# MCG-NKU/E2FGVI

Measured on AMD Instinct MI355X. Metric: inpainted frames/sec at 432x240 T=10, higher is better.
Workload: dtype f32; 1 GPU; BASELINE.json configs[1]: e2fgvi 432x240 T=10 l_t=10, 1 clip(s) per GPU per forward (1 in the job), random-init weights, torch.rand frames + box mask (SURVEY.md 8d); clips_per_gpu=1, precision=fp32, kernel_selection=e2fgvi_amd/tile_table.py (checked in, deterministic: ops.py), hip_graph=True, forwards_in_flight=2

## Files before the change

### e2fgvi_amd/build.py

```python
import os
import subprocess
import sys
from concurrent.futures import ThreadPoolExecutor

HERE = os.path.dirname(os.path.abspath(__file__))
CSRC = os.path.join(HERE, "csrc")
LIB = os.path.join(CSRC, "libe2fgvi_hip.so")
FLAGS = ["--offload-arch=gfx950", "-O3", "-std=c++17", "-fPIC", "-ffp-contract=fast"]
NOPK = ["-Xclang", "-target-feature", "-Xclang", "-packed-fp32-ops"]
UNITS = [("error.hip", "error.o", []), ("conv.hip", "conv.o", []), ("conv.hip", "conv_nopk.o", NOPK + ["-DE2_NOPK_VARIANT"]),
         ("conv_bf16x.hip", "conv_bf16x.o", NOPK), ("conv_wino.hip", "conv_wino.o", NOPK), ("conv_wino.hip", "conv_wino_x3.o", NOPK + ["-DE2_WINO_X3=1"]), ("conv_wino4.hip", "conv_wino4.o", NOPK), ("conv_tail.hip", "conv_tail.o", NOPK),
         ("mdcn.hip", "mdcn.o", NOPK), ("attention.hip", "attention.o", []),
         ("attention_bf16.hip", "attention_bf16.o", NOPK), ("attention_x3.hip", "attention_x3.o", NOPK), ("misc.hip", "misc.o", NOPK),
         ("video.hip", "video.o", NOPK), ("metrics.hip", "metrics.o", NOPK)]
NOPK_OBJECTS = ("conv_nopk.o", "conv_bf16x.o", "conv_wino.o", "conv_wino4.o", "conv_wino_x3.o", "conv_tail.o", "mdcn.o", "attention_bf16.o", "attention_x3.o", "misc.o", "video.o", "metrics.o")
OBJDUMP = "/opt/rocm/lib/llvm/bin/llvm-objdump"


def _hipcc():
    for c in (os.environ.get("HIPCC"), "/opt/rocm/bin/hipcc"):
        if c and os.path.exists(c):
            return c
    return "hipcc"


def _stale(out, deps):
    return (not os.path.exists(out)) or any(os.path.getmtime(d) > os.path.getmtime(out) for d in deps)


def build(force=False, verbose=False, nopk_all=False, lib=None, tag=None, defines=()):
    hipcc = _hipcc()
    if tag:
        nopk_all = False
    objdir = os.path.join(CSRC, ("build_" + tag) if tag else ("build_nopk" if nopk_all else "build"))
    os.makedirs(objdir, exist_ok=True)
    out = lib or (os.path.join(CSRC, "libe2fgvi_hip_%s.so" % tag) if tag else
                  os.path.join(CSRC, "libe2fgvi_hip_nopk.so") if nopk_all else LIB)
    headers = [os.path.join(CSRC, "common.h"), os.path.join(HERE, "..", "include", "e2fgvi_hip.h"), os.path.abspath(__file__)]
    jobs = []
    for src, obj, extra in UNITS:
        sp, op = os.path.join(CSRC, src), os.path.join(objdir, obj)
        if nopk_all and not any(f == "-packed-fp32-ops" for f in extra):
            extra = extra + NOPK
        if force or _stale(op, [sp] + headers):
            jobs.append([hipcc] + FLAGS + extra + list(defines) + ["-c", sp, "-o", op])

    def run(cmd):
        if verbose:
            print(" ".join(cmd), flush=True)
        subprocess.check_call(cmd)

    with ThreadPoolExecutor(max_workers=min(4, max(1, len(jobs)))) as ex:
        list(ex.map(run, jobs))
    objs = [os.path.join(objdir, obj) for _, obj, _ in UNITS]
    if force or jobs or _stale(out, objs):
        run([hipcc, "--offload-arch=gfx950", "-shared", "-fPIC", "-o", out] + objs)
    if jobs:
        verify_isa(objdir)
        if not nopk_all:
            verify_wino_waits(objdir)
            verify_exit_reuse(objdir)
            verify_no_scratch(objdir)
    return out


def build_variant(tag, *defines):
    return build(tag=tag, defines=defines)


def device_isa(obj):
    import shutil
    import tempfile
    d = tempfile.mkdtemp(prefix="e2isa")
    try:
        local = os.path.join(d, os.path.basename(obj))
        shutil.copy(obj, local)
        subprocess.run([OBJDUMP, "--offloading", os.path.basename(obj)], cwd=d, check=True, stdout=subprocess.DEVNULL,
                       stderr=subprocess.DEVNULL)
        dev = [f for f in os.listdir(d) if "gfx950" in f]
        if not dev:
            return ""
        return subprocess.run([OBJDUMP, "-d", os.path.join(d, dev[0])], check=True, capture_output=True, text=True).stdout
    finally:
        shutil.rmtree(d, ignore_errors=True)


def verify_isa(objdir=None):
    import re
    objdir = objdir or os.path.join(CSRC, "build")
    if not os.path.exists(OBJDUMP):
        return
    for obj in NOPK_OBJECTS:
        isa = device_isa(os.path.join(objdir, obj))
        bad = re.findall(r"v_pk_(?:mul|add|fma)_f32", isa)
        if bad or not isa:
# ... 273 lines not shown
```

### e2fgvi_amd/csrc/common.h

```cpp
#pragma once
#include <hip/hip_runtime.h>
#include <stdint.h>
#include <stdio.h>
#include <stdarg.h>

#include "../../include/e2fgvi_hip.h"

typedef float f32x4 __attribute__((ext_vector_type(4)));
typedef float f32x16 __attribute__((ext_vector_type(16)));

void e2fgvi_set_error(const char* fmt, ...);

#define E2_REQUIRE(cond, code, ...)            \
    do {                                       \
        if (!(cond)) {                         \
            e2fgvi_set_error(__VA_ARGS__);     \
            return (code);                     \
        }                                      \
    } while (0)

#define E2_LAUNCH_CHECK(name)                                                        \
    do {                                                                             \
        hipError_t e__ = hipGetLastError();                                          \
        if (e__ != hipSuccess) {                                                     \
// ... 54 lines not shown
typedef __bf16 e2_bf16x8 __attribute__((ext_vector_type(8)));
typedef unsigned int e2_u32x4 __attribute__((ext_vector_type(4)));
__device__ __forceinline__ void e2_split8(const f32x4& v0, const f32x4& v1, e2_bf16x8& hi, e2_bf16x8& mid, e2_bf16x8& lo) {
    float x[8];
#pragma unroll
    for (int j = 0; j < 4; ++j) { x[j] = v0[j]; x[4 + j] = v1[j]; }
    e2_u32x4 H, M, L;
#pragma unroll
    for (int j = 0; j < 4; ++j) {
        unsigned h, m, l;
        e2_split2(x[2 * j], x[2 * j + 1], h, m, l);
        H[j] = h; M[j] = m; L[j] = l;
    }
    hi = __builtin_bit_cast(e2_bf16x8, H);
    mid = __builtin_bit_cast(e2_bf16x8, M);
    lo = __builtin_bit_cast(e2_bf16x8, L);
}

typedef _Float16 e2_f16x8 __attribute__((ext_vector_type(8)));
template <bool F16> struct e2_h16;
template <> struct e2_h16<false> { typedef __bf16 T; typedef e2_bf16x8 V8; };
template <> struct e2_h16<true> { typedef _Float16 T; typedef e2_f16x8 V8; };
__device__ __forceinline__ f32x16 e2_mfma16(e2_bf16x8 a, e2_bf16x8 b, f32x16 c) {
    return __builtin_amdgcn_mfma_f32_32x32x16_bf16(a, b, c, 0, 0, 0);
}
__device__ __forceinline__ f32x16 e2_mfma16(e2_f16x8 a, e2_f16x8 b, f32x16 c) {
    return __builtin_amdgcn_mfma_f32_32x32x16_f16(a, b, c, 0, 0, 0);
}
template <bool F16> __device__ __forceinline__ float e2_h16_to_f32(unsigned short b) {
    if constexpr (F16) return (float)__builtin_bit_cast(_Float16, b);
    else return __builtin_bit_cast(float, (unsigned)b << 16);
}

__device__ __forceinline__ float apply_act(float v, int act, float slope) {
    if (act == E2FGVI_ACT_RELU) return fmaxf(v, 0.f);
    if (act == E2FGVI_ACT_LRELU) return v > 0.f ? v : v * slope;
    if (act == E2FGVI_ACT_TANH) return tanhf(v);
    return v;
}
```

### e2fgvi_amd/csrc/conv_bf16x.hip

```cpp
#include "common.h"

namespace {

typedef __bf16 bf16x8 __attribute__((ext_vector_type(8)));
typedef unsigned int u32x4 __attribute__((ext_vector_type(4)));
typedef __attribute__((address_space(3))) void lds_void;

struct ConvXParams {
    const void* src[E2FGVI_MAX_SRC];
    int ld[E2FGVI_MAX_SRC];
    int coff[E2FGVI_MAX_SRC];
    int cpg[E2FGVI_MAX_SRC];
    unsigned src_bytes[E2FGVI_MAX_SRC];
    int nsrc;
    int N, H, W, Ho, Wo, KH, KW, stride, pad;
    int padx;
    int osy, osx, opy, opx, oH, oW;
    int res_bcast;
    int Cout, Cout_g, Npad;
    int M;
    int tilesM, tilesN;
    int nsteps;
    unsigned wgroup_bytes;
    long long wgroup_elems;
    const void* w;
    const float* bias;
    const void* res;
    int res_ld, res_coff, res_bf16;
    void* dst;
    int dst_ld, dst_coff, dst_bf16, dst_nchw;
    __bf16* dst2;
    int dst2_ld, dst2_coff;
    int split_from;
    long long split_plane;
    int act;
    float slope;
    int tp_cq;
    unsigned tp_magic;
    unsigned tp_magic_cq;
    int dbg_noload;
};

__device__ __forceinline__ __amdgpu_buffer_rsrc_t make_rsrc(const void* base, unsigned bytes) {
    return __builtin_amdgcn_make_buffer_rsrc(const_cast<void*>(base), 0, (int)bytes, 0x00020000);
}

__device__ __forceinline__ float dcn_post(float v, int co, int C, const f32x4& fl, float max_residue) {
    const int noff = (C / 3) * 2;
    if (co >= noff) return e2_fast_sigmoid(v);
    const int which = (co * 2 >= noff) ? 2 : 0;
    return max_residue * e2_fast_tanh(v) + fl[which + ((co & 1) ? 0 : 1)];
}


__device__ __forceinline__ void split8(const f32x4& v0, const f32x4& v1, bf16x8& hi, bf16x8& mid, bf16x8& lo) {
    e2_split8(v0, v1, hi, mid, lo);
}

typedef int pp_i32x4 __attribute__((ext_vector_type(4)));
__device__ __forceinline__ pp_i32x4 pp_rsrc_words(const void* base, unsigned bytes) {
    const unsigned long long b = (unsigned long long)base;
    pp_i32x4 r;
    r[0] = __builtin_amdgcn_readfirstlane((int)(unsigned)b);
    r[1] = __builtin_amdgcn_readfirstlane((int)((unsigned)(b >> 32) & 0xFFFFu));
    r[2] = __builtin_amdgcn_readfirstlane((int)bytes);
    r[3] = 0x00020000;
    return r;
}
__device__ __forceinline__ void pp_dma16(pp_i32x4 rsrc, unsigned lds_dst, unsigned voff, unsigned soff) {
    unsigned keep;
    asm volatile("s_nop 4\n\ts_mov_b32 %0, m0\n\ts_mov_b32 m0, %3\n\ts_nop 0\n\tbuffer_load_dwordx4 %1, %2, %4 offen lds\n\ts_mov_b32 m0, %0"
                 : "=&s"(keep) : "v"(voff), "s"(rsrc), "s"(lds_dst), "s"(soff) : "memory");
}

template <int BM, int BN, int WGM, int WGN, bool S3, int MODE, bool PP = false>
__global__ __launch_bounds__(64 * WGM * WGN) void conv_bf16x_kernel(const ConvXParams p) {
#if defined(__HIP_DEVICE_COMPILE__)
    constexpr bool F32 = MODE == 1, X3 = MODE == 2, F16 = MODE == 3;
    typedef typename e2_h16<F16>::T E16;
    typedef typename e2_h16<F16>::V8 e16x8;
    static_assert(!PP || (X3 && !S3 && WGM * WGN == 8), "ping-pong halves: split-operand mode, 8 waves, no row-shift stages");
    constexpr int NT = 64 * WGM * WGN;
    constexpr int ESZ = (F32 || X3) ? 4 : 2;
    constexpr int CH = 16 / ESZ;
    constexpr int KC = 8 * CH;
    constexpr int TM = BM / (32 * WGM), TN = BN / (32 * WGN);
    constexpr int AR = S3 ? BM + 2 : BM;
    constexpr int B_CH = X3 ? 12 : 8;
    constexpr int A_BYTES = AR * 128, B_BYTES = BN * B_CH * 16;
    constexpr int A_IT = (AR * 8 + NT - 1) / NT, B_IT = (BN * B_CH + NT - 1) / NT;
    constexpr bool A_PART = (AR * 8) % NT != 0;
    constexpr bool B_PART = (BN * B_CH) % NT != 0;
    constexpr int R = TM * 32, CN = TN * 32;
    constexpr int ES = (WGM * WGN * R * (CN + 4) * 4 <= 150 * 1024) ? 1 : (TN % 2 == 0 ? 2 : TN);
    constexpr int TNH = TN / ES, CNH = CN / ES, LDE = CNH + 4;
    constexpr int EPI = WGM * WGN * R * LDE * 4;
    static_assert(TN % ES == 0 && EPI <= 160 * 1024, "epilogue region");
    constexpr int SMEM = 2 * (A_BYTES + B_BYTES) > EPI ? 2 * (A_BYTES + B_BYTES) : EPI;
    constexpr unsigned OOB = 0xFFFFFFFFu;
    static_assert(TM >= 1 && TN >= 1 && (BM * 8) % NT == 0 && (BN * B_CH) % 64 == 0 && SMEM <= 160 * 1024, "tile");

    __shared__ __attribute__((aligned(1024))) unsigned char smem[SMEM];

    const int tid = threadIdx.x;
    const int lane = tid & 63, wave = __builtin_amdgcn_readfirstlane(tid >> 6);
// ... 886 lines not shown
    p.wgroup_elems = q.wgroup_elems; p.wgroup_bytes = (unsigned)(q.wgroup_elems * wbytes_num);
    p.w = d->wpacked; p.bias = d->bias;
    p.res = d->residual; p.res_ld = d->res_ld; p.res_coff = d->res_coff; p.res_bf16 = d->res_dtype == dt16;
    p.dst = d->dst; p.dst_ld = d->dst_ld; p.dst_coff = d->dst_coff; p.dst_bf16 = d->dst_dtype == dt16;
    p.dst_nchw = d->dst_nchw;
    p.dst2 = (__bf16*)d->dst2; p.dst2_ld = d->dst2_ld; p.dst2_coff = d->dst2_coff;
    p.split_from = d->dst2_split_from; p.split_plane = d->dst2_plane_stride;
    p.act = d->act; p.slope = d->slope;
    hipStream_t st = (hipStream_t)stream;
    int tile = d->tile;
    p.dbg_noload = 0;
    if (tile == 21 || tile == 24 || tile == 26 || tile == 27) { p.dbg_noload = 1; tile -= 20; }
    if (tile == 31 || tile == 34 || tile == 36) { p.dbg_noload = 2; tile -= 30; }
    if (tile == 41 || tile == 44 || tile == 46) { p.dbg_noload = 3; tile -= 40; }
    if (tile == 61 || tile == 66) { p.dbg_noload = 8; tile -= 60; }
    if (tile == 71 || tile == 74 || tile == 76 || tile == 77) { p.dbg_noload = 16; tile -= 70; }
    if (tile == 81 || tile == 84 || tile == 86 || tile == 87) { p.dbg_noload = 32; tile -= 80; }
    if (!tile) {
        if (p.Cout_g <= 32) tile = 3;
        else if (p.Cout_g <= 64) tile = 2;
        else tile = ((long long)cdiv(p.M, 128) * cdiv(p.Cout_g, 128) * d->groups >= 384) ? 1 : 4;
    }
    switch (tile) {
        case 1: return launch_x<128, 128, 2, 2, false>(p, d->groups, st, mode);
        case 2: return launch_x<128, 64, 2, 2, false>(p, d->groups, st, mode);
        case 3: return launch_x<128, 32, 4, 1, false>(p, d->groups, st, mode);
        case 4: return launch_x<64, 128, 2, 2, false>(p, d->groups, st, mode);
        case 5: return launch_x<64, 64, 2, 2, false>(p, d->groups, st, mode);
        case 6: return launch_x<256, 128, 4, 2, false>(p, d->groups, st, mode);
        case 7: return launch_x<256, 256, 4, 2, false>(p, d->groups, st, mode);
        case 8: return launch_x<256, 192, 4, 2, false>(p, d->groups, st, mode);
        case 107: return launch_x<256, 256, 4, 2, false, true>(p, d->groups, st, mode);
        case 108: return launch_x<256, 192, 4, 2, false, true>(p, d->groups, st, mode);
        case 11: return launch_x<128, 128, 2, 2, true>(p, d->groups, st, mode);
        case 12: return launch_x<128, 64, 2, 2, true>(p, d->groups, st, mode);
        case 13: return launch_x<128, 32, 4, 1, true>(p, d->groups, st, mode);
        case 14: return launch_x<64, 128, 2, 2, true>(p, d->groups, st, mode);
        case 16: return launch_x<256, 128, 4, 2, true>(p, d->groups, st, mode);
        case 17: return launch_x<256, 256, 4, 2, true>(p, d->groups, st, mode);
        case 18: return launch_x<256, 64, 4, 2, true>(p, d->groups, st, mode);
        default: break;
    }
    e2fgvi_set_error("conv2d_x: unknown tile %d", tile);
    return E2FGVI_EINVAL;
}

extern "C" int e2fgvi_conv2d_x(const e2fgvi_convx_desc* d, int32_t mode, void* stream) {
    const int m = mode_x("conv2d_x", mode);
    return m < 0 ? E2FGVI_EINVAL : conv2d_x(d, stream, m);
}
```

### e2fgvi_amd/ops.py

```python
import ctypes as C
import math
import os

import torch

from . import lib as _L

ACT_NONE, ACT_RELU, ACT_LRELU, ACT_TANH, ACT_DCNPOST = _L.ACT_NONE, _L.ACT_RELU, _L.ACT_LRELU, _L.ACT_TANH, _L.ACT_DCNPOST


def _stream():
    return C.c_void_p(torch.cuda.current_stream().cuda_stream)


def _chk(t, name, dtype=torch.float32):
    if not isinstance(t, torch.Tensor) or not t.is_cuda:
        raise TypeError("%s must be a CUDA (ROCm) tensor -- the HIP path has no CPU fallback" % name)
    if t.dtype != dtype:
        raise TypeError("%s must be %s, got %s" % (name, dtype, t.dtype))
    if not t.is_contiguous():
        raise ValueError("%s must be contiguous" % name)
    return t


def _ptr(t):
    return C.c_void_p(t.data_ptr()) if t is not None else C.c_void_p(0)


def empty_nhwc(n, h, w, c, device):
    return torch.empty((n, h, w, c), dtype=torch.float32, device=device)


TUNE_CANDIDATES = (0, 213, 223, 211, 219, 216)
WINO_CANDIDATES = (64, 132, 164, 32)
W4_CODES = {2464: (2, 64)}
_W4_MINPIX = 20000
XTUNE_CANDIDATES = (1, 4, 6, 7, 8, 2, 5, 3, 107, 108)
XTUNE_ROWSHIFT = (11, 16, 17, 12, 13, 18)
X3_ENABLED = os.environ.get("E2FGVI_X3", "1") != "0"
X3_MARGIN = 0.97
X3_BASE = 30000
W3_BASE = 40000
W3_CANDIDATES = (132, 164, 32, 5132, 6064)
W3_WIDE = 6064
W3_WIDE_FALLBACK = 164
_TUNED = {}
AUTOTUNE = os.environ.get("E2FGVI_AUTOTUNE", "0") == "1"
TUNE_REPS = max(1, int(os.environ.get("E2FGVI_TUNE_REPS", "1") or 1))
TABLE_FORMAT = 2
_SIZE_FIELD = 8


def _default_tune_file():
    try:
        st = os.stat(_L.LIB_PATH)
        d = os.environ.get("E2FGVI_CACHE_DIR") or os.path.join(os.path.dirname(os.path.abspath(__file__)), ".tile_cache")
        os.makedirs(d, exist_ok=True)
        dev = "gpu"
        if torch.cuda.is_available():
            dev = "".join(ch for ch in torch.cuda.get_device_properties(0).gcnArchName.split(":")[0] if ch.isalnum())
        return os.path.join(d, "tiles_v%d_%s_%x_%x.txt" % (TABLE_FORMAT, dev, st.st_size, int(st.st_mtime)))
    except (OSError, RuntimeError):
        return None


_TUNE_FILE = None
if AUTOTUNE:
    _TUNE_FILE = os.environ.get("E2FGVI_TUNE_FILE")
    if _TUNE_FILE is None:
        _TUNE_FILE = _default_tune_file()
# ... 662 lines not shown
                     out2=None if out2 is None else out2[n0:n1], tile=tile, out_nchw=out_nchw)
            return out
        d = self._desc(srcs, out, out_coff, residual, res_coff, act, slope, out2, out_nchw)
        if planes is not None:
            self._set_planes(d, planes, split_from, N * Ho * Wo)
        d.tile = tile
        x3 = self.try_x3 and X3_ENABLED and self.f32 and not self.x3
        if tile == 0 and self.tune and N * Ho * Wo >= 2048:
            key = (("x3" if self.x3 else ("x32+3" if x3 else "x32")) if self.f32 else "x", self.Cout, tuple(self.cpg), self.KH, self.KW, self.stride, self.pad, self.groups,
                   int(4.0 * math.log2(N * Ho * Wo)), _dt_key(out), out_nchw, self.taps)
            best = _decision(key)
            if best is None and AUTOTUNE and not torch.cuda.is_current_stream_capturing() and (
                    residual is None or residual.data_ptr() != out.data_ptr()):
                res = self._time_tiles(d)
                best = min(res, key=res.get) if res else 0
                if x3 and self._alt3() is not None:
                    res3 = self.alt3._time_tiles(self.alt3._desc(srcs, out, out_coff, residual, res_coff, act, slope, out2, out_nchw))
                    if res3 and (not res or min(res3.values()) < X3_MARGIN * min(res.values())):
                        best = X3_BASE + min(res3, key=res3.get)
                best = _remember(key, best)
            if best and best >= X3_BASE and self._alt3() is not None:
                try:
                    return self.alt3(srcs, out=out, out_dtype=out_dtype, out_coff=out_coff, residual=residual, res_coff=res_coff, act=act,
                                     slope=slope, out2=out2, tile=best - X3_BASE, out_nchw=out_nchw, planes=planes, split_from=split_from)
                except _L.HipError:
                    best = 0
            d.tile = tile = (best or 0) if (best or 0) < X3_BASE else 0
        if _L.TRACE is not None:
            cin_g, cout_g, K2 = sum(self.cpg), self.Cout // self.groups, self.KH * self.KW
            kc = 32 if self.f32 else 64
            cin_p = sum(-(-c // kc) * kc for c in self.cpg)
            if self.taps:
                cin_p = -(-K2 * (self.cpg[0] // (4 if self.f32 else 8)) // 8) * kc / K2
            _L.annotate(layer=self.name, kernel="conv_%s tile=%d%s" % (("f32x3" if self.x3 else "f32x") if self.f32 else
                                                                      "f16x" if self.f16 else "bf16x", tile,
                                                                      " taps" if self.taps else ""),
                        shape="N%d %dx%d %d->%d k%d s%d g%d" % (N, H, W, cin_g * self.groups, self.Cout, self.KH, self.stride, self.groups),
                        macs=N * Ho * Wo * self.Cout * cin_g * K2,
                        issued=int(N * Ho * Wo * (-(-cout_g // 32) * 32) * self.groups * cin_p * K2 * (6 * 157.3 / 2500.0 if self.x3 else 1)))
        d.wpacked = self.wpacked.data_ptr()
        rc = self._fn(C.byref(d), _stream())
        if rc != 0 and d.tile and self.tune:
            d.tile = 0
            rc = self._fn(C.byref(d), _stream())
        _L.check(rc, "conv2d_x")
        return out

    def _time_tiles(self, d, reps=3, rounds=2):
        st = _stream()
        res = {}
        d.tile = 0
        d.wpacked = self.wpacked.data_ptr()
        for _ in range(2):
            self._fn(C.byref(d), st)
        for _ in range(rounds * TUNE_REPS):
            rowshift = (self.KH, self.KW, self.stride, self.pad) == (3, 3, 1, 1) and not self.f32 and not self.taps
            for code in XTUNE_CANDIDATES + (XTUNE_ROWSHIFT if rowshift else ()):
                if code % 10 == 3 and self.Cout // self.groups > 64:
                    continue
                if code in (12, 18) and self.Cout // self.groups > 64:
                    continue
                d.tile = code
                if self._fn(C.byref(d), st) != 0:
                    continue
                e0, e1 = torch.cuda.Event(enable_timing=True), torch.cuda.Event(enable_timing=True)
                e0.record()
                for _ in range(reps):
                    self._fn(C.byref(d), st)
                e1.record()
                e1.synchronize()
                res[code] = min(res.get(code, float("inf")), e0.elapsed_time(e1) / reps)
        d.tile = 0
# ... 661 lines not shown
```

### e2fgvi_amd/tile_table.py

```python
TABLE_FORMAT = 2
TILES = {
    ('x', 128, (128, 128), 1, 1, 1, 0, 1, 63, 1, False, False): 1,
    ('x', 128, (128, 128), 1, 1, 1, 0, 1, 76, 1, False, False): 4,
    ('x', 128, (128, 128), 1, 1, 1, 0, 1, 85, 1, False, False): 4,
    ('x', 128, (128, 128), 3, 3, 1, 1, 1, 50, 1, False, False): 5,
    ('x', 128, (128, 128), 3, 3, 1, 1, 1, 63, 1, False, False): 1,
    ('x', 128, (128, 128), 3, 3, 1, 1, 1, 68, 1, False, False): 4,
    ('x', 128, (128, 128, 128), 3, 3, 1, 1, 1, 50, 1, False, False): 5,
    ('x', 128, (128, 128, 128), 3, 3, 1, 1, 1, 63, 1, False, False): 11,
    ('x', 128, (128, 128, 128), 3, 3, 1, 1, 1, 68, 1, False, False): 4,
    ('x', 128, (128, 128, 128, 8), 3, 3, 1, 1, 1, 50, 1, False, False): 5,
    ('x', 128, (128, 128, 128, 8), 3, 3, 1, 1, 1, 63, 1, False, False): 11,
    ('x', 128, (128, 128, 128, 8), 3, 3, 1, 1, 1, 68, 1, False, False): 11,
    ('x', 128, (128,), 3, 3, 1, 1, 1, 50, 1, False, False): 5,
    ('x', 128, (128,), 3, 3, 1, 1, 1, 63, 1, False, False): 6,
    ('x', 128, (128,), 3, 3, 1, 1, 1, 68, 1, False, False): 4,
    ('x', 128, (128,), 3, 3, 1, 1, 1, 71, 1, False, False): 1,
    ('x', 128, (128,), 3, 3, 1, 1, 1, 76, 1, False, False): 1,
    ('x', 128, (128,), 3, 3, 1, 1, 1, 84, 1, False, False): 1,
    ('x', 128, (128,), 3, 3, 1, 1, 1, 85, 1, False, False): 6,
    ('x', 128, (128,), 3, 3, 1, 1, 1, 93, 1, False, False): 6,
    ('x', 128, (256, 256), 3, 3, 1, 1, 1, 63, 1, False, False): 16,
    ('x', 128, (256, 256), 3, 3, 1, 1, 1, 76, 1, False, False): 11,
    ('x', 128, (256, 256), 3, 3, 1, 1, 1, 85, 1, False, False): 11,
# ... 227 lines not shown
    (2, (16,), 7, 7, 1, 3, 1, 16, 48, True, 0, False, False, 0, 'x3'): 0,
    (2, (16,), 7, 7, 1, 3, 1, 16, 49, True, 0, False, False, 0, 'x3'): 0,
    (2, (16,), 7, 7, 1, 3, 1, 16, 52, True, 0, False, False, 0, 'x3'): 0,
    (2, (16,), 7, 7, 1, 3, 1, 16, 53, True, 0, False, False, 0, 'x3'): 0,
    (2, (16,), 7, 7, 1, 3, 1, 16, 56, True, 0, False, False, 0, 'x3'): 0,
    (2, (16,), 7, 7, 1, 3, 1, 16, 57, True, 0, False, False, 0, 'x3'): 0,
    (2, (16,), 7, 7, 1, 3, 1, 16, 60, True, 0, False, False, 0, 'x3'): 0,
    (2, (16,), 7, 7, 1, 3, 1, 16, 61, True, 0, False, False, 0, 'x3'): 0,
    (2, (16,), 7, 7, 1, 3, 1, 16, 64, True, 0, False, False, 0, 'x3'): 0,
    (2, (16,), 7, 7, 1, 3, 1, 16, 65, True, 0, False, False, 0, 'x3'): 0,
    (2, (16,), 7, 7, 1, 3, 1, 16, 68, True, 0, False, False, 0, 'x3'): 0,
    (2, (16,), 7, 7, 1, 3, 1, 16, 69, True, 0, False, False, 0, 'x3'): 0,
    (2, (16,), 7, 7, 1, 3, 1, 16, 72, True, 0, False, False, 0, 'x3'): 0,
    (2, (16,), 7, 7, 1, 3, 1, 16, 73, True, 0, False, False, 0, 'x3'): 0,
    (2, (16,), 7, 7, 1, 3, 1, 16, 80, True, 0, False, False, 0, 'x3'): 0,
    (256, (128,), 3, 3, 1, 1, 1, 32, 59, False, 2, True, False, 0, 'x3'): 45132,
    (256, (128,), 3, 3, 1, 1, 1, 32, 63, False, 2, True, False, 0, 'x3'): 46064,
    (256, (128,), 3, 3, 1, 1, 1, 32, 67, False, 2, True, False, 0, 'x3'): 46064,
    (256, (128,), 3, 3, 1, 1, 1, 32, 68, False, 2, True, False, 0, 'x3'): 46064,
    (256, (128,), 3, 3, 1, 1, 1, 32, 75, False, 2, True, False, 0, 'x3'): 46064,
    (256, (32, 48), 3, 3, 1, 1, 8, 16, 59, False, 2, True, False, 0, 'x3'): 0,
    (256, (32, 48), 3, 3, 1, 1, 8, 16, 63, False, 2, True, False, 0, 'x3'): 45132,
    (256, (32, 48), 3, 3, 1, 1, 8, 16, 67, False, 2, True, False, 0, 'x3'): 0,
    (256, (32, 48), 3, 3, 1, 1, 8, 16, 68, False, 2, True, False, 0, 'x3'): 0,
    (256, (32, 48), 3, 3, 1, 1, 8, 16, 75, False, 2, True, False, 0, 'x3'): 0,
    (32, (64,), 7, 7, 1, 3, 1, 32, 44, False, 1, False, False, 0, 'x3'): 0,
    (32, (64,), 7, 7, 1, 3, 1, 32, 45, False, 1, False, False, 0, 'x3'): 0,
    (32, (64,), 7, 7, 1, 3, 1, 32, 48, False, 1, False, False, 0, 'x3'): 0,
    (32, (64,), 7, 7, 1, 3, 1, 32, 49, False, 1, False, False, 0, 'x3'): 0,
    (32, (64,), 7, 7, 1, 3, 1, 32, 52, False, 1, False, False, 0, 'x3'): 0,
    (32, (64,), 7, 7, 1, 3, 1, 32, 53, False, 1, False, False, 0, 'x3'): 0,
    (32, (64,), 7, 7, 1, 3, 1, 32, 56, False, 1, False, False, 0, 'x3'): 0,
    (32, (64,), 7, 7, 1, 3, 1, 32, 57, False, 1, False, False, 0, 'x3'): 0,
    (32, (64,), 7, 7, 1, 3, 1, 32, 60, False, 1, False, False, 0, 'x3'): 30003,
    (32, (64,), 7, 7, 1, 3, 1, 32, 61, False, 1, False, False, 0, 'x3'): 30003,
    (32, (64,), 7, 7, 1, 3, 1, 32, 64, False, 1, False, False, 0, 'x3'): 30003,
    (32, (64,), 7, 7, 1, 3, 1, 32, 65, False, 1, False, False, 0, 'x3'): 30003,
    (32, (64,), 7, 7, 1, 3, 1, 32, 68, False, 1, False, False, 0, 'x3'): 30003,
    (32, (64,), 7, 7, 1, 3, 1, 32, 69, False, 1, False, False, 0, 'x3'): 30003,
    (32, (64,), 7, 7, 1, 3, 1, 32, 72, False, 1, False, False, 0, 'x3'): 30003,
    (32, (64,), 7, 7, 1, 3, 1, 32, 73, False, 1, False, False, 0, 'x3'): 30003,
    (32, (64,), 7, 7, 1, 3, 1, 32, 80, False, 1, False, False, 0, 'x3'): 30003,
    (32, (8,), 7, 7, 1, 3, 1, 8, 44, False, 1, False, False, 0, 'x3'): 0,
    (32, (8,), 7, 7, 1, 3, 1, 8, 45, False, 1, False, False, 0, 'x3'): 0,
    (32, (8,), 7, 7, 1, 3, 1, 8, 48, False, 1, False, False, 0, 'x3'): 0,
    (32, (8,), 7, 7, 1, 3, 1, 8, 49, False, 1, False, False, 0, 'x3'): 0,
    (32, (8,), 7, 7, 1, 3, 1, 8, 52, False, 1, False, False, 0, 'x3'): 0,
    (32, (8,), 7, 7, 1, 3, 1, 8, 53, False, 1, False, False, 0, 'x3'): 0,
    (32, (8,), 7, 7, 1, 3, 1, 8, 56, False, 1, False, False, 0, 'x3'): 0,
    (32, (8,), 7, 7, 1, 3, 1, 8, 57, False, 1, False, False, 0, 'x3'): 0,
    (32, (8,), 7, 7, 1, 3, 1, 8, 60, False, 1, False, False, 0, 'x3'): 0,
    (32, (8,), 7, 7, 1, 3, 1, 8, 61, False, 1, False, False, 0, 'x3'): 0,
    (32, (8,), 7, 7, 1, 3, 1, 8, 64, False, 1, False, False, 0, 'x3'): 0,
    (32, (8,), 7, 7, 1, 3, 1, 8, 65, False, 1, False, False, 0, 'x3'): 0,
    (32, (8,), 7, 7, 1, 3, 1, 8, 68, False, 1, False, False, 0, 'x3'): 0,
    (32, (8,), 7, 7, 1, 3, 1, 8, 69, False, 1, False, False, 0, 'x3'): 0,
    (32, (8,), 7, 7, 1, 3, 1, 8, 72, False, 1, False, False, 0, 'x3'): 0,
    (32, (8,), 7, 7, 1, 3, 1, 8, 73, False, 1, False, False, 0, 'x3'): 0,
    (32, (8,), 7, 7, 1, 3, 1, 8, 80, False, 1, False, False, 0, 'x3'): 0,
    (384, (256,), 3, 3, 1, 1, 1, 32, 59, False, 2, True, False, 2464, 'x3'): 46064,
    (384, (256,), 3, 3, 1, 1, 1, 32, 63, False, 2, True, False, 2464, 'x3'): 46064,
    (384, (256,), 3, 3, 1, 1, 1, 32, 67, False, 2, True, False, 2464, 'x3'): 46064,
    (384, (256,), 3, 3, 1, 1, 1, 32, 68, False, 2, True, False, 0, 'x3'): 46064,
    (384, (256,), 3, 3, 1, 1, 1, 32, 75, False, 2, True, False, 2464, 'x3'): 46064,
    (384, (64, 128), 3, 3, 1, 1, 4, 32, 59, False, 2, True, False, 0, 'x3'): 45132,
    (384, (64, 128), 3, 3, 1, 1, 4, 32, 63, False, 2, True, False, 0, 'x3'): 45132,
    (384, (64, 128), 3, 3, 1, 1, 4, 32, 67, False, 2, True, False, 0, 'x3'): 45132,
    (384, (64, 128), 3, 3, 1, 1, 4, 32, 68, False, 2, True, False, 0, 'x3'): 46064,
    (384, (64, 128), 3, 3, 1, 1, 4, 32, 75, False, 2, True, False, 0, 'x3'): 46064,
    (432, (128,), 3, 3, 1, 1, 1, 32, 50, True, 4, True, False, 0, 'x3'): 46064,
    (432, (128,), 3, 3, 1, 1, 1, 32, 54, True, 4, True, False, 0, 'x3'): 46064,
# ... 22 lines not shown
    (512, (512,), 1, 1, 1, 0, 1, 32, 47, True, 0, False, True, 0): 2005,
    (512, (512,), 1, 1, 1, 0, 1, 32, 47, True, 0, False, True, 0, 'x3'): 30005,
    (512, (512,), 1, 1, 1, 0, 1, 32, 51, True, 0, False, True, 0): 2004,
    (512, (512,), 1, 1, 1, 0, 1, 32, 51, True, 0, False, True, 0, 'x3'): 30004,
    (512, (512,), 1, 1, 1, 0, 1, 32, 54, True, 0, False, True, 0): 2005,
    (512, (512,), 1, 1, 1, 0, 1, 32, 54, True, 0, False, True, 0, 'x3'): 30001,
    (512, (512,), 1, 1, 1, 0, 1, 32, 55, True, 0, False, True, 0): 2001,
    (512, (512,), 1, 1, 1, 0, 1, 32, 55, True, 0, False, True, 0, 'x3'): 30001,
    (512, (512,), 1, 1, 1, 0, 1, 32, 63, True, 0, False, True, 0): 2005,
    (512, (512,), 1, 1, 1, 0, 1, 32, 63, True, 0, False, True, 0, 'x3'): 30107,
    (6272, (512,), 1, 1, 1, 0, 1, 32, 47, False, 0, False, True, 0): 2004,
    (6272, (512,), 1, 1, 1, 0, 1, 32, 47, False, 0, False, True, 0, 'x3'): 30108,
    (6272, (512,), 1, 1, 1, 0, 1, 32, 51, False, 0, False, True, 0): 2004,
    (6272, (512,), 1, 1, 1, 0, 1, 32, 51, False, 0, False, True, 0, 'x3'): 30107,
    (6272, (512,), 1, 1, 1, 0, 1, 32, 54, False, 0, False, True, 0): 2007,
    (6272, (512,), 1, 1, 1, 0, 1, 32, 54, False, 0, False, True, 0, 'x3'): 30107,
    (6272, (512,), 1, 1, 1, 0, 1, 32, 55, False, 0, False, True, 0): 2002,
    (6272, (512,), 1, 1, 1, 0, 1, 32, 55, False, 0, False, True, 0, 'x3'): 30107,
    (6272, (512,), 1, 1, 1, 0, 1, 32, 63, False, 0, False, True, 0): 2007,
    (6272, (512,), 1, 1, 1, 0, 1, 32, 63, False, 0, False, True, 0, 'x3'): 30107,
    (64, (128,), 3, 3, 1, 1, 1, 32, 67, False, 2, True, False, 0, 'x3'): 46064,
    (64, (128,), 3, 3, 1, 1, 1, 32, 71, False, 2, True, False, 0, 'x3'): 46064,
    (64, (128,), 3, 3, 1, 1, 1, 32, 75, False, 2, True, False, 0, 'x3'): 46064,
    (64, (128,), 3, 3, 1, 1, 1, 32, 76, False, 2, True, False, 0, 'x3'): 46064,
    (64, (128,), 3, 3, 1, 1, 1, 32, 83, False, 2, True, False, 0, 'x3'): 46064,
    (64, (32,), 7, 7, 1, 3, 1, 32, 44, False, 1, False, False, 0, 'x3'): 0,
    (64, (32,), 7, 7, 1, 3, 1, 32, 45, False, 1, False, False, 0, 'x3'): 0,
    (64, (32,), 7, 7, 1, 3, 1, 32, 48, False, 1, False, False, 0, 'x3'): 0,
    (64, (32,), 7, 7, 1, 3, 1, 32, 49, False, 1, False, False, 0, 'x3'): 0,
    (64, (32,), 7, 7, 1, 3, 1, 32, 52, False, 1, False, False, 0, 'x3'): 0,
    (64, (32,), 7, 7, 1, 3, 1, 32, 53, False, 1, False, False, 0, 'x3'): 0,
    (64, (32,), 7, 7, 1, 3, 1, 32, 56, False, 1, False, False, 0, 'x3'): 0,
    (64, (32,), 7, 7, 1, 3, 1, 32, 57, False, 1, False, False, 0, 'x3'): 30005,
    (64, (32,), 7, 7, 1, 3, 1, 32, 60, False, 1, False, False, 0, 'x3'): 30005,
    (64, (32,), 7, 7, 1, 3, 1, 32, 61, False, 1, False, False, 0, 'x3'): 30005,
    (64, (32,), 7, 7, 1, 3, 1, 32, 64, False, 1, False, False, 0, 'x3'): 30002,
    (64, (32,), 7, 7, 1, 3, 1, 32, 65, False, 1, False, False, 0, 'x3'): 30005,
    (64, (32,), 7, 7, 1, 3, 1, 32, 68, False, 1, False, False, 0, 'x3'): 30005,
    (64, (32,), 7, 7, 1, 3, 1, 32, 69, False, 1, False, False, 0, 'x3'): 30005,
    (64, (32,), 7, 7, 1, 3, 1, 32, 72, False, 1, False, False, 0, 'x3'): 30005,
    (64, (32,), 7, 7, 1, 3, 1, 32, 73, False, 1, False, False, 0, 'x3'): 30005,
    (64, (32,), 7, 7, 1, 3, 1, 32, 80, False, 1, False, False, 0, 'x3'): 30005,
    (64, (4,), 3, 3, 2, 1, 1, 8, 67, False, 2, False, False, 0, 'x3'): 0,
    (64, (4,), 3, 3, 2, 1, 1, 8, 71, False, 2, False, False, 0, 'x3'): 0,
    (64, (4,), 3, 3, 2, 1, 1, 8, 75, False, 2, False, False, 0, 'x3'): 0,
    (64, (4,), 3, 3, 2, 1, 1, 8, 76, False, 2, False, False, 0, 'x3'): 0,
    (64, (4,), 3, 3, 2, 1, 1, 8, 83, False, 2, False, False, 0, 'x3'): 0,
    (64, (64,), 3, 3, 1, 1, 1, 32, 67, False, 2, True, False, 0, 'x3'): 45132,
    (64, (64,), 3, 3, 1, 1, 1, 32, 71, False, 2, True, False, 0, 'x3'): 45132,
    (64, (64,), 3, 3, 1, 1, 1, 32, 75, False, 2, True, False, 0, 'x3'): 45132,
    (64, (64,), 3, 3, 1, 1, 1, 32, 76, False, 2, True, False, 0, 'x3'): 46064,
    (64, (64,), 3, 3, 1, 1, 1, 32, 79, False, 2, True, False, 0, 'x3'): 46064,
    (64, (64,), 3, 3, 1, 1, 1, 32, 83, False, 2, True, False, 0, 'x3'): 46064,
    (64, (64,), 3, 3, 1, 1, 1, 32, 84, False, 2, True, False, 0, 'x3'): 46064,
    (64, (64,), 3, 3, 1, 1, 1, 32, 91, False, 2, True, False, 0, 'x3'): 46064,
}
```

Before: 955.1 frames/s.

## Add halo-staged split-bf16 direct conv kernel for 7x7 stride-1 layers

Adds a new direct-convolution kernel for 7x7 stride-1 pad-3 layers. For each 8x32 output tile it stages the haloed input patch in LDS once as three bf16 split planes (hi, mid, lo) and reuses that patch across all 49 taps, instead of going through an im2col-style GEMM. Weights are double-buffered through LDS with buffer-load-to-LDS DMA, and the products use six bf16 MFMAs per k-step to emulate fp32. The tile table routes a few small-Cout 7x7 layers (roughly 32-64 channels) to tiles 201 and 202. The cost is a barrier per tap and some padded compute at tile edges.

```diff
diff --git a/e2fgvi_amd/build.py b/e2fgvi_amd/build.py
--- a/e2fgvi_amd/build.py
+++ b/e2fgvi_amd/build.py
@@ -9,11 +9,11 @@
 FLAGS = ["--offload-arch=gfx950", "-O3", "-std=c++17", "-fPIC", "-ffp-contract=fast"]
 NOPK = ["-Xclang", "-target-feature", "-Xclang", "-packed-fp32-ops"]
 UNITS = [("error.hip", "error.o", []), ("conv.hip", "conv.o", []), ("conv.hip", "conv_nopk.o", NOPK + ["-DE2_NOPK_VARIANT"]),
-         ("conv_bf16x.hip", "conv_bf16x.o", NOPK), ("conv_wino.hip", "conv_wino.o", NOPK), ("conv_wino.hip", "conv_wino_x3.o", NOPK + ["-DE2_WINO_X3=1"]), ("conv_wino4.hip", "conv_wino4.o", NOPK), ("conv_tail.hip", "conv_tail.o", NOPK),
+         ("conv_bf16x.hip", "conv_bf16x.o", NOPK), ("conv_halo_x3.hip", "conv_halo_x3.o", NOPK), ("conv_wino.hip", "conv_wino.o", NOPK), ("conv_wino.hip", "conv_wino_x3.o", NOPK + ["-DE2_WINO_X3=1"]), ("conv_wino4.hip", "conv_wino4.o", NOPK), ("conv_tail.hip", "conv_tail.o", NOPK),
          ("mdcn.hip", "mdcn.o", NOPK), ("attention.hip", "attention.o", []),
          ("attention_bf16.hip", "attention_bf16.o", NOPK), ("attention_x3.hip", "attention_x3.o", NOPK), ("misc.hip", "misc.o", NOPK),
          ("video.hip", "video.o", NOPK), ("metrics.hip", "metrics.o", NOPK)]
-NOPK_OBJECTS = ("conv_nopk.o", "conv_bf16x.o", "conv_wino.o", "conv_wino4.o", "conv_wino_x3.o", "conv_tail.o", "mdcn.o", "attention_bf16.o", "attention_x3.o", "misc.o", "video.o", "metrics.o")
+NOPK_OBJECTS = ("conv_nopk.o", "conv_bf16x.o", "conv_halo_x3.o", "conv_wino.o", "conv_wino4.o", "conv_wino_x3.o", "conv_tail.o", "mdcn.o", "attention_bf16.o", "attention_x3.o", "misc.o", "video.o", "metrics.o")
 OBJDUMP = "/opt/rocm/lib/llvm/bin/llvm-objdump"
 
 
@@ -61,6 +61,7 @@
             verify_wino_waits(objdir)
             verify_exit_reuse(objdir)
             verify_no_scratch(objdir)
+            verify_no_scratch(objdir, "conv_halo_x3.o", "conv_halo_x3_kernel")
     return out
 
 
diff --git a/e2fgvi_amd/csrc/common.h b/e2fgvi_amd/csrc/common.h
--- a/e2fgvi_amd/csrc/common.h
+++ b/e2fgvi_amd/csrc/common.h
@@ -110,6 +110,24 @@
     else return __builtin_bit_cast(float, (unsigned)b << 16);
 }
 
+typedef int pp_i32x4 __attribute__((ext_vector_type(4)));
+__device__ __forceinline__ pp_i32x4 pp_rsrc_words(const void* base, unsigned bytes) {
+    const unsigned long long b = (unsigned long long)base;
+    pp_i32x4 r;
+    r[0] = __builtin_amdgcn_readfirstlane((int)(unsigned)b);
+    r[1] = __builtin_amdgcn_readfirstlane((int)((unsigned)(b >> 32) & 0xFFFFu));
+    r[2] = __builtin_amdgcn_readfirstlane((int)bytes);
+    r[3] = 0x00020000;
+    return r;
+}
+__device__ __forceinline__ void pp_dma16(pp_i32x4 rsrc, unsigned lds_dst, unsigned voff, unsigned soff) {
+    unsigned keep;
+    asm volatile("s_nop 4\n\ts_mov_b32 %0, m0\n\ts_mov_b32 m0, %3\n\ts_nop 0\n\tbuffer_load_dwordx4 %1, %2, %4 offen lds\n\ts_mov_b32 m0, %0"
+                 : "=&s"(keep) : "v"(voff), "s"(rsrc), "s"(lds_dst), "s"(soff) : "memory");
+}
+
+int e2_conv_halo_x3(const e2fgvi_convx_desc* d, int tile, hipStream_t st);
+
 __device__ __forceinline__ float apply_act(float v, int act, float slope) {
     if (act == E2FGVI_ACT_RELU) return fmaxf(v, 0.f);
     if (act == E2FGVI_ACT_LRELU) return v > 0.f ? v : v * slope;
diff --git a/e2fgvi_amd/csrc/conv_bf16x.hip b/e2fgvi_amd/csrc/conv_bf16x.hip
--- a/e2fgvi_amd/csrc/conv_bf16x.hip
+++ b/e2fgvi_amd/csrc/conv_bf16x.hip
@@ -55,22 +55,6 @@
 
 __device__ __forceinline__ void split8(const f32x4& v0, const f32x4& v1, bf16x8& hi, bf16x8& mid, bf16x8& lo) {
     e2_split8(v0, v1, hi, mid, lo);
-}
-
-typedef int pp_i32x4 __attribute__((ext_vector_type(4)));
-__device__ __forceinline__ pp_i32x4 pp_rsrc_words(const void* base, unsigned bytes) {
-    const unsigned long long b = (unsigned long long)base;
-    pp_i32x4 r;
-    r[0] = __builtin_amdgcn_readfirstlane((int)(unsigned)b);
-    r[1] = __builtin_amdgcn_readfirstlane((int)((unsigned)(b >> 32) & 0xFFFFu));
-    r[2] = __builtin_amdgcn_readfirstlane((int)bytes);
-    r[3] = 0x00020000;
-    return r;
-}
-__device__ __forceinline__ void pp_dma16(pp_i32x4 rsrc, unsigned lds_dst, unsigned voff, unsigned soff) {
-    unsigned keep;
-    asm volatile("s_nop 4\n\ts_mov_b32 %0, m0\n\ts_mov_b32 m0, %3\n\ts_nop 0\n\tbuffer_load_dwordx4 %1, %2, %4 offen lds\n\ts_mov_b32 m0, %0"
-                 : "=&s"(keep) : "v"(voff), "s"(rsrc), "s"(lds_dst), "s"(soff) : "memory");
 }
 
 template <int BM, int BN, int WGM, int WGN, bool S3, int MODE, bool PP = false>
@@ -1023,6 +1007,9 @@
         case 8: return launch_x<256, 192, 4, 2, false>(p, d->groups, st, mode);
         case 107: return launch_x<256, 256, 4, 2, false, true>(p, d->groups, st, mode);
         case 108: return launch_x<256, 192, 4, 2, false, true>(p, d->groups, st, mode);
+        case 201: case 202:
+            E2_REQUIRE(mode == 2, E2FGVI_EUNSUP, "conv2d_x: the halo-staged tiles (201, 202) are for the split-operand mode");
+            return e2_conv_halo_x3(d, tile, st);
         case 11: return launch_x<128, 128, 2, 2, true>(p, d->groups, st, mode);
         case 12: return launch_x<128, 64, 2, 2, true>(p, d->groups, st, mode);
         case 13: return launch_x<128, 32, 4, 1, true>(p, d->groups, st, mode);
diff --git a/e2fgvi_amd/csrc/conv_halo_x3.hip b/e2fgvi_amd/csrc/conv_halo_x3.hip
--- /dev/null
+++ b/e2fgvi_amd/csrc/conv_halo_x3.hip
@@ -0,0 +1,253 @@
+#include "common.h"
+
+namespace {
+
+typedef __bf16 bf16x8 __attribute__((ext_vector_type(8)));
+typedef __attribute__((address_space(3))) void lds_void;
+
+struct HaloX3Params {
+    const float* src[E2FGVI_MAX_SRC];
+    int ld[E2FGVI_MAX_SRC], coff[E2FGVI_MAX_SRC], cpg[E2FGVI_MAX_SRC];
+    int nsrc, nchunks;
+    int N, H, W;
+    int Cout, Npad;
+    int tilesY, tilesX;
+    unsigned wbytes;
+    const void* w;
+    const float* bias;
+    const float* res;
+    int res_ld, res_coff;
+    float* dst;
+    int dst_ld, dst_coff;
+    int act;
+    float slope;
+};
+
+constexpr int HX_K = 7, HX_PAD = 3, HX_TH = 8, HX_TW = 32;
+constexpr int HX_PH = HX_TH + HX_K - 1, HX_PW = HX_TW + HX_K - 1, HX_NPIX = HX_PH * HX_PW;
+
+template <int TN>
+__global__ __launch_bounds__(512) void conv_halo_x3_kernel(const HaloX3Params p) {
+#if defined(__HIP_DEVICE_COMPILE__)
+    constexpr int NT = 512, BN = 32 * TN;
+    constexpr int PLANE = HX_NPIX * 64;
+    constexpr int B_ITEMS = BN * 12, B_BYTES = B_ITEMS * 16;
+    constexpr int B_IT = (B_ITEMS + NT - 1) / NT;
+    constexpr int P_ITEMS = HX_NPIX * 4, P_IT = (P_ITEMS + NT - 1) / NT;
+    constexpr int LDE = BN + 4, EPI = 8 * 32 * LDE * 4;
+    constexpr int SMEM = 2 * B_BYTES + 3 * PLANE > EPI ? 2 * B_BYTES + 3 * PLANE : EPI;
+    constexpr unsigned OOB = 0xFFFFFFFFu;
+    static_assert(SMEM <= 160 * 1024 && B_ITEMS % 64 == 0 && (2 * B_BYTES) % 1024 == 0, "LDS layout");
+
+    __shared__ __attribute__((aligned(1024))) unsigned char smem[SMEM];
+    unsigned char* const planes = smem + 2 * B_BYTES;
+
+    const int tid = threadIdx.x;
+    const int lane = tid & 63, wave = __builtin_amdgcn_readfirstlane(tid >> 6);
+    const int i = lane & 31, h = lane >> 5;
+    const int per_img = p.tilesY * p.tilesX;
+    const int logical = xcd_remap(blockIdx.x, p.N * per_img);
+    const int img = logical / per_img;
+    const int trem = logical - img * per_img;
+    const int ty = trem / p.tilesX, tx = trem - ty * p.tilesX;
+    const int y0 = ty * HX_TH, x0 = tx * HX_TW;
+
+    int g_pix[P_IT];
+    int l_off[P_IT];
+#pragma unroll
+    for (int it = 0; it < P_IT; ++it) {
+        const int item = tid + it * NT;
+        const int pix = item >> 2, q = item & 3;
+        const int py = pix / HX_PW, px = pix - py * HX_PW;
+        const int iy = y0 - HX_PAD + py, ix = x0 - HX_PAD + px;
+        const bool in = item < P_ITEMS && (unsigned)iy < (unsigned)p.H && (unsigned)ix < (unsigned)p.W;
+        g_pix[it] = in ? (img * p.H + iy) * p.W + ix : -1;
+        l_off[it] = item < P_ITEMS ? pix * 64 + ((q ^ ((pix >> 2) & 3)) << 4) : -1;
+    }
+    unsigned b_off[B_IT];
+#pragma unroll
+    for (int it = 0; it < B_IT; ++it) {
+        const int item = tid + it * NT;
+        const int ch = item / BN, n = item - ch * BN;
+        b_off[it] = (n < p.Npad && ch < 12) ? (unsigned)((ch * p.Npad + n) * 16) : OOB;
+    }
+    const unsigned b_step = 12u * (unsigned)p.Npad * 16u;
+    const pp_i32x4 wrsrc = pp_rsrc_words(p.w, p.wbytes);
+    const unsigned smem_lds = (unsigned)(unsigned long long)(lds_void*)smem;
+    auto issue_b = [&](int stage, int step) __attribute__((always_inline)) {
+        const unsigned lb = smem_lds + (unsigned)(stage * B_BYTES + wave * 1024);
+        const unsigned sb = (unsigned)__builtin_amdgcn_readfirstlane((int)((unsigned)step * b_step));
+#pragma unroll
+        for (int it = 0; it < B_IT; ++it)
+            if (tid + it * NT < B_ITEMS)
+                pp_dma16(wrsrc, (unsigned)__builtin_amdgcn_readfirstlane((int)(lb + it * NT * 16)), b_off[it], sb);
+    };
+
+    f32x16 acc[TN];
+#pragma unroll
+    for (int tn = 0; tn < TN; ++tn)
+#pragma unroll
+        for (int r = 0; r < 16; ++r) acc[tn][r] = 0.f;
+
+    const int pbase = wave * HX_PW + i;
+    int b_rd[TN];
+#pragma unroll
+    for (int tn = 0; tn < TN; ++tn) b_rd[tn] = (tn * 32 + i) * 16;
+
+    const float* const sp0 = p.src[0]; const float* const sp1 = p.src[1]; const float* const sp2 = p.src[2]; const float* const sp3 = p.src[3];
+    int s = 0, c0 = 0;
+    for (int ck = 0; ck < p.nchunks; ++ck) {
+        const float* const sp = s == 0 ? sp0 : s == 1 ? sp1 : s == 2 ? sp2 : sp3;
+        const int ld = p.ld[s], cpg = p.cpg[s];
+        const int cfirst = p.coff[s] + c0;
+        const int noct = (cpg - c0 >= 32) ? 4 : (cpg - c0) >> 3;
+        issue_b(0, ck);
+        {
+            f32x4 v0[P_IT], v1[P_IT];
+#pragma unroll
+            for (int it = 0; it < P_IT; ++it) {
+                const int q = (tid + it * NT) & 3;
+                const f32x4 z = {0.f, 0.f, 0.f, 0.f};
+                v0[it] = z; v1[it] = z;
+                if (g_pix[it] >= 0 && q < noct) {
+                    const float* g = sp + (long long)g_pix[it] * ld + cfirst + q * 8;
+                    v0[it] = *reinterpret_cast<const f32x4*>(g);
+                    v1[it] = *reinterpret_cast<const f32x4*>(g + 4);
+                }
+            }
+#pragma unroll
+            for (int it = 0; it < P_IT; ++it) {
+                bf16x8 hi, mid, lo;
+                e2_split8(v0[it], v1[it], hi, mid, lo);
+                if (l_off[it] >= 0) {
+                    *reinterpret_cast<bf16x8*>(planes + l_off[it]) = hi;
+                    *reinterpret_cast<bf16x8*>(planes + PLANE + l_off[it]) = mid;
+                    *reinterpret_cast<bf16x8*>(planes + 2 * PLANE + l_off[it]) = lo;
+                }
+            }
+        }
+        asm volatile("s_waitcnt vmcnt(0)" ::: "memory");
+        __syncthreads();
+        int ky = 0, kx = 0;
+        for (int tap = 0; tap < HX_K * HX_K; ++tap) {
+            const int cur = tap & 1;
+            if (tap + 1 < HX_K * HX_K) issue_b(cur ^ 1, (tap + 1) * p.nchunks + ck);
+            const unsigned char* const stb = smem + cur * B_BYTES;
+            const int pp = pbase + ky * HX_PW + kx;
+            const unsigned char* const ap = planes + pp * 64;
+            const int key = (pp >> 2) & 3;
+#pragma unroll
+            for (int kk = 0; kk < 2; ++kk) {
+                if (kk == 1 && noct <= 2) break;
+                const int q = 2 * kk + h;
+                const int ao = (q ^ key) << 4;
+                const bf16x8 ah = *reinterpret_cast<const bf16x8*>(ap + ao);
+                const bf16x8 am = *reinterpret_cast<const bf16x8*>(ap + PLANE + ao);
+                const bf16x8 al = *reinterpret_cast<const bf16x8*>(ap + 2 * PLANE + ao);
+#pragma unroll
+                for (int tn = 0; tn < TN; ++tn) {
+                    const bf16x8 bh = *reinterpret_cast<const bf16x8*>(stb + b_rd[tn] + q * (BN * 16));
+                    const bf16x8 bm = *reinterpret_cast<const bf16x8*>(stb + b_rd[tn] + (4 + q) * (BN * 16));
+                    const bf16x8 bl = *reinterpret_cast<const bf16x8*>(stb + b_rd[tn] + (8 + q) * (BN * 16));
+                    acc[tn] = __builtin_amdgcn_mfma_f32_32x32x16_bf16(al, bh, acc[tn], 0, 0, 0);
+                    acc[tn] = __builtin_amdgcn_mfma_f32_32x32x16_bf16(ah, bl, acc[tn], 0, 0, 0);
+                    acc[tn] = __builtin_amdgcn_mfma_f32_32x32x16_bf16(am, bm, acc[tn], 0, 0, 0);
+                    acc[tn] = __builtin_amdgcn_mfma_f32_32x32x16_bf16(am, bh, acc[tn], 0, 0, 0);
+                    acc[tn] = __builtin_amdgcn_mfma_f32_32x32x16_bf16(ah, bm, acc[tn], 0, 0, 0);
+                    acc[tn] = __builtin_amdgcn_mfma_f32_32x32x16_bf16(ah, bh, acc[tn], 0, 0, 0);
+                }
+            }
+            asm volatile("s_waitcnt vmcnt(0)" ::: "memory");
+            __syncthreads();
+            if (++kx == HX_K) { kx = 0; ++ky; }
+        }
+        c0 += 32;
+        if (c0 >= cpg) { c0 = 0; ++s; }
+    }
+
+    float* E = reinterpret_cast<float*>(smem) + wave * (32 * LDE);
+#pragma unroll
+    for (int tn = 0; tn < TN; ++tn)
+#pragma unroll
+        for (int r = 0; r < 16; ++r)
+            E[((r & 3) + 8 * (r >> 2) + 4 * h) * LDE + tn * 32 + i] = acc[tn][r];
+    __syncthreads();
+    constexpr int LPR = BN / 4, RPP = 64 / LPR;
+    const int co = (lane % LPR) * 4;
+    const int oy = y0 + wave;
+    if (co >= p.Cout || oy >= p.H) return;
+    const bool full = co + 3 < p.Cout;
+    float bv[4];
+#pragma unroll
+    for (int c = 0; c < 4; ++c) bv[c] = (p.bias && (full || co + c < p.Cout)) ? p.bias[co + c] : 0.f;
+    const bool vec_d = full && ((p.dst_ld | p.dst_coff) & 3) == 0;
+    const bool vec_r = full && ((p.res_ld | p.res_coff) & 3) == 0;
+#pragma unroll 1
+    for (int ps = 0; ps < 32 / RPP; ++ps) {
+        const int rr = ps * RPP + lane / LPR;
+        const int ox = x0 + rr;
+        if (ox >= p.W) continue;
+        const long long m = ((long long)img * p.H + oy) * p.W + ox;
+        const f32x4 e = *reinterpret_cast<const f32x4*>(E + rr * LDE + co);
+        float v[4] = {e[0] + bv[0], e[1] + bv[1], e[2] + bv[2], e[3] + bv[3]};
+        if (p.res) {
+            const float* rp = p.res + m * p.res_ld + p.res_coff + co;
+            if (vec_r) {
+                const f32x4 r4 = *reinterpret_cast<const f32x4*>(rp);
+#pragma unroll
+                for (int c = 0; c < 4; ++c) v[c] += r4[c];
+            } else {
+#pragma unroll
+                for (int c = 0; c < 4; ++c) if (full || co + c < p.Cout) v[c] += rp[c];
+            }
+        }
+#pragma unroll
+        for (int c = 0; c < 4; ++c) v[c] = apply_act(v[c], p.act, p.slope);
+        float* o = p.dst + m * p.dst_ld + p.dst_coff + co;
+        if (vec_d) {
+            const f32x4 w4 = {v[0], v[1], v[2], v[3]};
+            *reinterpret_cast<f32x4*>(o) = w4;
+        } else {
+#pragma unroll
+            for (int c = 0; c < 4; ++c) if (full || co + c < p.Cout) o[c] = v[c];
+        }
+    }
+#endif
+}
+
+}
+
+int e2_conv_halo_x3(const e2fgvi_convx_desc* d, int tile, hipStream_t st) {
+    const int tn = tile - 200;
+    E2_REQUIRE(tn == 1 || tn == 2, E2FGVI_EINVAL, "conv_halo_x3: unknown tile %d", tile);
+    E2_REQUIRE(d->KH == HX_K && d->KW == HX_K && d->stride == 1 && d->pad == HX_PAD && !d->out_grid, E2FGVI_EUNSUP,
+               "conv_halo_x3: tiles 201 / 202 are for 7x7 stride-1 pad-3 layers (got %dx%d stride %d pad %d)", d->KH, d->KW, d->stride, d->pad);
+    E2_REQUIRE(d->groups == 1 && !d->tap_packed, E2FGVI_EUNSUP, "conv_halo_x3: no groups, no tap-packed weights");
+    E2_REQUIRE(d->Cout <= 32 * tn, E2FGVI_EUNSUP, "conv_halo_x3: tile %d takes at most %d output channels (got %d)", tile, 32 * tn, d->Cout);
+    E2_REQUIRE(!d->dst_nchw && d->dst_dtype == E2FGVI_F32 && !d->dst2 && !d->dst2_plane_stride && !d->res_bcast &&
+               (!d->residual || d->res_dtype == E2FGVI_F32) && d->act <= E2FGVI_ACT_LRELU, E2FGVI_EUNSUP,
+               "conv_halo_x3: fp32 NHWC dst and residual, no second copy, activation none / ReLU / LeakyReLU");
+    HaloX3Params p;
+    p.nchunks = 0;
+    for (int s = 0; s < E2FGVI_MAX_SRC; ++s) { p.src[s] = nullptr; p.ld[s] = 0; p.coff[s] = 0; p.cpg[s] = 0; }
+    for (int s = 0; s < d->nsrc; ++s) {
+        E2_REQUIRE(d->src_cpg[s] % 8 == 0, E2FGVI_EUNSUP, "conv_halo_x3: source %d has %d channels, not a multiple of 8", s, d->src_cpg[s]);
+        p.src[s] = static_cast<const float*>(d->src[s]); p.ld[s] = d->src_ld[s]; p.coff[s] = d->src_coff[s]; p.cpg[s] = d->src_cpg[s];
+        p.nchunks += cdiv(d->src_cpg[s], 32);
+    }
+    p.nsrc = d->nsrc;
+    p.N = d->N; p.H = d->H; p.W = d->W;
+    p.Cout = d->Cout; p.Npad = round_up(d->Cout, 32);
+    p.tilesY = cdiv(d->H, HX_TH); p.tilesX = cdiv(d->W, HX_TW);
+    E2_REQUIRE((long long)d->N * p.tilesY * p.tilesX < 2147483647LL, E2FGVI_EUNSUP, "conv_halo_x3: more than 2^31 tiles");
+    p.wbytes = (unsigned)((long long)HX_K * HX_K * p.nchunks * 32 * p.Npad * 6);
+    p.w = d->wpacked; p.bias = d->bias;
+    p.res = static_cast<const float*>(d->residual); p.res_ld = d->res_ld; p.res_coff = d->res_coff;
+    p.dst = static_cast<float*>(d->dst); p.dst_ld = d->dst_ld; p.dst_coff = d->dst_coff;
+    p.act = d->act; p.slope = d->slope;
+    const dim3 grid((unsigned)(d->N * p.tilesY * p.tilesX)), block(512);
+    if (tn == 1) hipLaunchKernelGGL(conv_halo_x3_kernel<1>, grid, block, 0, st, p);
+    else hipLaunchKernelGGL(conv_halo_x3_kernel<2>, grid, block, 0, st, p);
+    E2_LAUNCH_CHECK("conv_halo_x3");
+    return 0;
+}
diff --git a/e2fgvi_amd/ops.py b/e2fgvi_amd/ops.py
--- a/e2fgvi_amd/ops.py
+++ b/e2fgvi_amd/ops.py
@@ -35,7 +35,8 @@
 WINO_CANDIDATES = (64, 132, 164, 32)
 W4_CODES = {2464: (2, 64)}
 _W4_MINPIX = 20000
-XTUNE_CANDIDATES = (1, 4, 6, 7, 8, 2, 5, 3, 107, 108)
+XTUNE_CANDIDATES = (1, 4, 6, 7, 8, 2, 5, 3, 107, 108, 201, 202)
+HALO_X3_TILES = (201, 202)
 XTUNE_ROWSHIFT = (11, 16, 17, 12, 13, 18)
 X3_ENABLED = os.environ.get("E2FGVI_X3", "1") != "0"
 X3_MARGIN = 0.97
@@ -764,12 +765,17 @@
             cin_p = sum(-(-c // kc) * kc for c in self.cpg)
             if self.taps:
                 cin_p = -(-K2 * (self.cpg[0] // (4 if self.f32 else 8)) // 8) * kc / K2
-            _L.annotate(layer=self.name, kernel="conv_%s tile=%d%s" % (("f32x3" if self.x3 else "f32x") if self.f32 else
-                                                                      "f16x" if self.f16 else "bf16x", tile,
-                                                                      " taps" if self.taps else ""),
+            pix, cout_p = N * Ho * Wo, -(-cout_g // 32) * 32
+            kern = "conv_%s tile=%d%s" % (("f32x3" if self.x3 else "f32x") if self.f32 else "f16x" if self.f16 else "bf16x", tile,
+                                          " taps" if self.taps else "")
+            if self.x3 and tile in HALO_X3_TILES:
+                pix, cout_p = N * (-(-Ho // 8) * 8) * (-(-Wo // 32) * 32), 32 * (tile - 200)
+                cin_p = sum(c // 32 * 32 + (-(-(c % 32) // 16) * 16) for c in self.cpg)
+                kern = "conv_halo_x3<%d>" % cout_p
+            _L.annotate(layer=self.name, kernel=kern,
                         shape="N%d %dx%d %d->%d k%d s%d g%d" % (N, H, W, cin_g * self.groups, self.Cout, self.KH, self.stride, self.groups),
                         macs=N * Ho * Wo * self.Cout * cin_g * K2,
-                        issued=int(N * Ho * Wo * (-(-cout_g // 32) * 32) * self.groups * cin_p * K2 * (6 * 157.3 / 2500.0 if self.x3 else 1)))
+                        issued=int(pix * cout_p * self.groups * cin_p * K2 * (6 * 157.3 / 2500.0 if self.x3 else 1)))
         d.wpacked = self.wpacked.data_ptr()
         rc = self._fn(C.byref(d), _stream())
         if rc != 0 and d.tile and self.tune:
diff --git a/e2fgvi_amd/tile_table.py b/e2fgvi_amd/tile_table.py
--- a/e2fgvi_amd/tile_table.py
+++ b/e2fgvi_amd/tile_table.py
@@ -283,11 +283,11 @@
     (32, (64,), 7, 7, 1, 3, 1, 32, 53, False, 1, False, False, 0, 'x3'): 0,
     (32, (64,), 7, 7, 1, 3, 1, 32, 56, False, 1, False, False, 0, 'x3'): 0,
     (32, (64,), 7, 7, 1, 3, 1, 32, 57, False, 1, False, False, 0, 'x3'): 0,
-    (32, (64,), 7, 7, 1, 3, 1, 32, 60, False, 1, False, False, 0, 'x3'): 30003,
+    (32, (64,), 7, 7, 1, 3, 1, 32, 60, False, 1, False, False, 0, 'x3'): 30201,
     (32, (64,), 7, 7, 1, 3, 1, 32, 61, False, 1, False, False, 0, 'x3'): 30003,
     (32, (64,), 7, 7, 1, 3, 1, 32, 64, False, 1, False, False, 0, 'x3'): 30003,
     (32, (64,), 7, 7, 1, 3, 1, 32, 65, False, 1, False, False, 0, 'x3'): 30003,
-    (32, (64,), 7, 7, 1, 3, 1, 32, 68, False, 1, False, False, 0, 'x3'): 30003,
+    (32, (64,), 7, 7, 1, 3, 1, 32, 68, False, 1, False, False, 0, 'x3'): 30201,
     (32, (64,), 7, 7, 1, 3, 1, 32, 69, False, 1, False, False, 0, 'x3'): 30003,
     (32, (64,), 7, 7, 1, 3, 1, 32, 72, False, 1, False, False, 0, 'x3'): 30003,
     (32, (64,), 7, 7, 1, 3, 1, 32, 73, False, 1, False, False, 0, 'x3'): 30003,
@@ -376,11 +376,11 @@
     (64, (32,), 7, 7, 1, 3, 1, 32, 53, False, 1, False, False, 0, 'x3'): 0,
     (64, (32,), 7, 7, 1, 3, 1, 32, 56, False, 1, False, False, 0, 'x3'): 0,
     (64, (32,), 7, 7, 1, 3, 1, 32, 57, False, 1, False, False, 0, 'x3'): 30005,
-    (64, (32,), 7, 7, 1, 3, 1, 32, 60, False, 1, False, False, 0, 'x3'): 30005,
+    (64, (32,), 7, 7, 1, 3, 1, 32, 60, False, 1, False, False, 0, 'x3'): 30202,
     (64, (32,), 7, 7, 1, 3, 1, 32, 61, False, 1, False, False, 0, 'x3'): 30005,
     (64, (32,), 7, 7, 1, 3, 1, 32, 64, False, 1, False, False, 0, 'x3'): 30002,
     (64, (32,), 7, 7, 1, 3, 1, 32, 65, False, 1, False, False, 0, 'x3'): 30005,
-    (64, (32,), 7, 7, 1, 3, 1, 32, 68, False, 1, False, False, 0, 'x3'): 30005,
+    (64, (32,), 7, 7, 1, 3, 1, 32, 68, False, 1, False, False, 0, 'x3'): 30202,
     (64, (32,), 7, 7, 1, 3, 1, 32, 69, False, 1, False, False, 0, 'x3'): 30005,
     (64, (32,), 7, 7, 1, 3, 1, 32, 72, False, 1, False, False, 0, 'x3'): 30005,
     (64, (32,), 7, 7, 1, 3, 1, 32, 73, False, 1, False, False, 0, 'x3'): 30005,
```

Result: no change. 961.3 frames/s, median of 2 (+0.6%).
